# Gadersd/stable-diffusion-xl-burn

Hardware: NVIDIA H100
Metric: unet_sampler_steps_per_sec_1024x1024_bs1 (higher is better)
Workload: dtype f16

## Files before the change

### stable-diffusion-xl-burn_b200/csrc/attention.cu

```cuda
#include <stdlib.h>

#include "common.cuh"
#include "kernels.h"

namespace sdxl {

static constexpr int kTileBytes = 128 * 128;
static constexpr int kKvStages = 3;
static constexpr int kConsumerWarps = 8;
static constexpr int kAttnThreads = kConsumerWarps * 32 + 32;
static constexpr int kAttnSmem = 1024  + kTileBytes + 2 * kKvStages * kTileBytes + 256;

__device__ __forceinline__ float ex2_approx(float x) {
  float y;
  asm("ex2.approx.ftz.f32 %0, %1;" : "=f"(y) : "f"(x));
  return y;
}
__device__ __forceinline__ uint32_t pack_half2(float a, float b) {
  __half2 t = __floats2half2_rn(a, b);
  return *reinterpret_cast<uint32_t*>(&t);
}

__global__ void __launch_bounds__(kAttnThreads, 1) attention_kernel(const __grid_constant__ AttnParams p) {
  extern __shared__ uint8_t smem_raw[];
  uint8_t* smem = reinterpret_cast<uint8_t*>((reinterpret_cast<uintptr_t>(smem_raw) + 1023) & ~uintptr_t(1023));
  uint8_t* sQ = smem;
  uint8_t* sK = sQ + kTileBytes;
  uint8_t* sV = sK + kKvStages * kTileBytes;
  uint64_t* bars = reinterpret_cast<uint64_t*>(sV + kKvStages * kTileBytes);
  uint64_t* q_full = bars;
  uint64_t* kv_full = q_full + 1;
  uint64_t* kv_empty = kv_full + kKvStages;

  const int warp = threadIdx.x >> 5, lane = threadIdx.x & 31;
  const int nblk = (p.S + 127) / 128;
  const int nqt = (p.T + 127) / 128;
  const int qt = blockIdx.x % nqt, head = (blockIdx.x / nqt) % p.n_head, b = blockIdx.x / (nqt * p.n_head);

  if (threadIdx.x == 0) {
    tma_prefetch_desc(&p.tmQ);
    tma_prefetch_desc(&p.tmK);
    tma_prefetch_desc(&p.tmV);
    mbar_init(q_full, 1);
    for (int i = 0; i < kKvStages; ++i) { mbar_init(&kv_full[i], 1); mbar_init(&kv_empty[i], kConsumerWarps); }
    fence_barrier_init();
  }
  __syncthreads();
  griddep_wait();
  griddep_launch_dependents();

  if (warp == kConsumerWarps) {
    if (lane != 0) return;
    mbar_expect_tx(q_full, kTileBytes);
    tma_load_3d(sQ, &p.tmQ, q_full, p.q_col0 + head * 64, qt * 128, b);
    for (int j = 0; j < nblk; ++j) {
      const int st = j % kKvStages;
      mbar_wait_nocall(&kv_empty[st], ((j / kKvStages) & 1) ^ 1);
      mbar_expect_tx(&kv_full[st], 2 * kTileBytes);
      tma_load_3d(sK + st * kTileBytes, &p.tmK, &kv_full[st], p.k_col0 + head * 64, j * 128, b);
      tma_load_3d(sV + st * kTileBytes, &p.tmV, &kv_full[st], p.v_col0 + head * 64, j * 128, b);
    }
    return;
  }

  const int wg = warp >> 2;
  const float sl2e = p.scale_log2e;
  const uint32_t q_addr = smem_u32(sQ) + (uint32_t)wg * (64 * 128);
  float o[32];
#pragma unroll
  for (int i = 0; i < 32; ++i) o[i] = 0.f;
  float m[2] = {-INFINITY, -INFINITY}, l[2] = {0.f, 0.f};
  mbar_wait_nocall(q_full, 0);
  for (int j = 0; j < nblk; ++j) {
    const int st = j % kKvStages;
    mbar_wait_nocall(&kv_full[st], (j / kKvStages) & 1);
    float s[64];
    wg_fence();
    const uint32_t k_addr = smem_u32(sK + st * kTileBytes);
#pragma unroll
    for (int k = 0; k < 4; ++k) wgmma_ss_n128(s, wg_desc_sw128(q_addr + 32 * k), wg_desc_sw128(k_addr + 32 * k), k);
    wg_commit();
    wg_wait<0>();
    if (j * 128 + 128 > p.S) {
#pragma unroll
      for (int jj = 0; jj < 16; ++jj)
#pragma unroll
        for (int e = 0; e < 2; ++e)
          if (j * 128 + 8 * jj + 2 * (lane & 3) + e >= p.S) { s[4 * jj + e] = -INFINITY; s[4 * jj + 2 + e] = -INFINITY; }
    }
    uint32_t pa[32];
#pragma unroll
    for (int h = 0; h < 2; ++h) {
      float mx = -INFINITY;
#pragma unroll
      for (int jj = 0; jj < 16; ++jj) mx = fmaxf(mx, fmaxf(s[4 * jj + 2 * h], s[4 * jj + 2 * h + 1]));
      mx = fmaxf(mx, __shfl_xor_sync(0xffffffffu, mx, 1));
      mx = fmaxf(mx, __shfl_xor_sync(0xffffffffu, mx, 2));
      const float m_new = fmaxf(m[h], mx);
      const float alpha = ex2_approx((m[h] - m_new) * sl2e);
      const float mb = m_new * sl2e;
      float sum = 0.f;
#pragma unroll
      for (int jj = 0; jj < 16; ++jj) {
        const float p0 = ex2_approx(fmaf(s[4 * jj + 2 * h], sl2e, -mb));
        const float p1 = ex2_approx(fmaf(s[4 * jj + 2 * h + 1], sl2e, -mb));
        sum += p0 + p1;
        pa[4 * (jj >> 1) + 2 * (jj & 1) + h] = pack_half2(p0, p1);
      }
      l[h] = l[h] * alpha + sum;
      m[h] = m_new;
#pragma unroll
      for (int jj = 0; jj < 8; ++jj) { o[4 * jj + 2 * h] *= alpha; o[4 * jj + 2 * h + 1] *= alpha; }
    }
    wg_fence();
    const uint32_t v_addr = smem_u32(sV + st * kTileBytes);
#pragma unroll
    for (int kk = 0; kk < 8; ++kk)
      wgmma_rs_n64_tb(o, *reinterpret_cast<const uint32_t(*)[4]>(pa + 4 * kk), wg_desc_sw128(v_addr + 2048 * kk));
    wg_commit();
    wg_wait<0>();
    if (lane == 0) mbar_arrive(&kv_empty[st]);
  }
  const int r = wg * 64 + (warp & 3) * 16 + (lane >> 2);
#pragma unroll
  for (int h = 0; h < 2; ++h) {
    float lt = l[h];
    lt += __shfl_xor_sync(0xffffffffu, lt, 1);
    lt += __shfl_xor_sync(0xffffffffu, lt, 2);
    const float inv = 1.0f / lt;
    const int t = qt * 128 + r + 8 * h;
    if (t < p.T) {
      __half* out = p.out + ((size_t)b * p.T + t) * p.ldo + head * 64 + 2 * (lane & 3);
#pragma unroll
      for (int jj = 0; jj < 8; ++jj)
        *reinterpret_cast<__half2*>(out + 8 * jj) = __floats2half2_rn(o[4 * jj + 2 * h] * inv, o[4 * jj + 2 * h + 1] * inv);
    }
  }
}

static bool g_attn_attr[64];
int attention_launch(cudaStream_t st, const AttnParams& p) {
  if (p.T < 1 || p.S < 1 || (p.ldo & 1)) return 2002;
  int r = smem_optin(attention_kernel, kAttnSmem, g_attn_attr);
  if (r) return r;
  const long tiles = (long)p.B * p.n_head * ((p.T + 127) / 128);
  return launch_kernel(attention_kernel, dim3((unsigned)tiles), dim3(kAttnThreads), (size_t)kAttnSmem, st, true, p);
}

}
```

Before: 27.62.

## Make attention persistent with double-buffered Q and overlapped QK/PV wgmma

Turns the attention kernel into a persistent kernel sized to the SM count. It double-buffers Q tiles and keeps K/V resident across consecutive query tiles when the key length fits in one block (cross-attention). Inside the key loop, the next QK^T wgmma is issued alongside the previous block's PV wgmma so softmax overlaps tensor-core work. It also widens the producer to a full warpgroup with setmaxnreg rebalancing and adds a fourth KV stage, at the cost of more shared memory and more complex barrier phase tracking.

```diff
diff --git a/stable-diffusion-xl-burn_b200/csrc/attention.cu b/stable-diffusion-xl-burn_b200/csrc/attention.cu
--- a/stable-diffusion-xl-burn_b200/csrc/attention.cu
+++ b/stable-diffusion-xl-burn_b200/csrc/attention.cu
@@ -6,10 +6,9 @@
 namespace sdxl {
 
 static constexpr int kTileBytes = 128 * 128;
-static constexpr int kKvStages = 3;
-static constexpr int kConsumerWarps = 8;
-static constexpr int kAttnThreads = kConsumerWarps * 32 + 32;
-static constexpr int kAttnSmem = 1024  + kTileBytes + 2 * kKvStages * kTileBytes + 256;
+static constexpr int kKvStages = 4;
+static constexpr int kAttnThreads = 3 * 128;
+static constexpr int kAttnSmem = 1024  + 2 * kTileBytes + 2 * kKvStages * kTileBytes + 256;
 
 __device__ __forceinline__ float ex2_approx(float x) {
   float y;
@@ -21,27 +20,99 @@
   return *reinterpret_cast<uint32_t*>(&t);
 }
 
+__device__ __forceinline__ void softmax_block(float (&s)[64], float (&m)[2], float (&l)[2], float (&alpha)[2], int j, int S,
+                                              float sl2e, int lane) {
+  if (j * 128 + 128 > S) {
+#pragma unroll
+    for (int jj = 0; jj < 16; ++jj)
+#pragma unroll
+      for (int e = 0; e < 2; ++e)
+        if (j * 128 + 8 * jj + 2 * (lane & 3) + e >= S) { s[4 * jj + e] = -INFINITY; s[4 * jj + 2 + e] = -INFINITY; }
+  }
+#pragma unroll
+  for (int h = 0; h < 2; ++h) {
+    float mx = -INFINITY;
+#pragma unroll
+    for (int jj = 0; jj < 16; ++jj) mx = fmaxf(mx, fmaxf(s[4 * jj + 2 * h], s[4 * jj + 2 * h + 1]));
+    mx = fmaxf(mx, __shfl_xor_sync(0xffffffffu, mx, 1));
+    mx = fmaxf(mx, __shfl_xor_sync(0xffffffffu, mx, 2));
+    const float m_new = fmaxf(m[h], mx);
+    alpha[h] = ex2_approx((m[h] - m_new) * sl2e);
+    const float mb = m_new * sl2e;
+    float sum = 0.f;
+#pragma unroll
+    for (int jj = 0; jj < 16; ++jj) {
+      const float p0 = ex2_approx(fmaf(s[4 * jj + 2 * h], sl2e, -mb));
+      const float p1 = ex2_approx(fmaf(s[4 * jj + 2 * h + 1], sl2e, -mb));
+      sum += p0 + p1;
+      s[4 * jj + 2 * h] = p0;
+      s[4 * jj + 2 * h + 1] = p1;
+    }
+    l[h] = l[h] * alpha[h] + sum;
+    m[h] = m_new;
+  }
+}
+__device__ __forceinline__ void rescale_pack(float (&o)[32], const float (&s)[64], uint32_t (&pa)[32], const float (&alpha)[2]) {
+#pragma unroll
+  for (int h = 0; h < 2; ++h) {
+#pragma unroll
+    for (int jj = 0; jj < 8; ++jj) { o[4 * jj + 2 * h] *= alpha[h]; o[4 * jj + 2 * h + 1] *= alpha[h]; }
+#pragma unroll
+    for (int jj = 0; jj < 16; ++jj) pa[4 * (jj >> 1) + 2 * (jj & 1) + h] = pack_half2(s[4 * jj + 2 * h], s[4 * jj + 2 * h + 1]);
+  }
+}
+__device__ __forceinline__ void issue_s(float (&s)[64], uint32_t q_addr, uint32_t k_addr) {
+#pragma unroll
+  for (int k = 0; k < 4; ++k) wgmma_ss_n128(s, wg_desc_sw128(q_addr + 32 * k), wg_desc_sw128(k_addr + 32 * k), k);
+  wg_commit();
+}
+__device__ __forceinline__ void issue_pv(float (&o)[32], const uint32_t (&pa)[32], uint32_t v_addr) {
+#pragma unroll
+  for (int kk = 0; kk < 8; ++kk)
+    wgmma_rs_n64_tb(o, *reinterpret_cast<const uint32_t(*)[4]>(pa + 4 * kk), wg_desc_sw128(v_addr + 2048 * kk));
+  wg_commit();
+}
+
+struct TileWalk {
+  int nblk, nqt, t0, end, step;
+  bool resident;
+  __device__ TileWalk(const AttnParams& p) {
+    nblk = (p.S + 127) / 128;
+    nqt = (p.T + 127) / 128;
+    resident = nblk == 1;
+    const int tiles = p.B * p.n_head * nqt;
+    if (resident) {
+      t0 = (int)((long long)blockIdx.x * tiles / gridDim.x);
+      end = (int)((long long)(blockIdx.x + 1) * tiles / gridDim.x);
+      step = 1;
+    } else {
+      t0 = blockIdx.x;
+      end = tiles;
+      step = gridDim.x;
+    }
+  }
+};
+
 __global__ void __launch_bounds__(kAttnThreads, 1) attention_kernel(const __grid_constant__ AttnParams p) {
   extern __shared__ uint8_t smem_raw[];
   uint8_t* smem = reinterpret_cast<uint8_t*>((reinterpret_cast<uintptr_t>(smem_raw) + 1023) & ~uintptr_t(1023));
   uint8_t* sQ = smem;
-  uint8_t* sK = sQ + kTileBytes;
+  uint8_t* sK = sQ + 2 * kTileBytes;
   uint8_t* sV = sK + kKvStages * kTileBytes;
   uint64_t* bars = reinterpret_cast<uint64_t*>(sV + kKvStages * kTileBytes);
   uint64_t* q_full = bars;
-  uint64_t* kv_full = q_full + 1;
+  uint64_t* q_empty = q_full + 2;
+  uint64_t* kv_full = q_empty + 2;
   uint64_t* kv_empty = kv_full + kKvStages;
+  constexpr int kConsumerWarps = 8;
 
   const int warp = threadIdx.x >> 5, lane = threadIdx.x & 31;
-  const int nblk = (p.S + 127) / 128;
-  const int nqt = (p.T + 127) / 128;
-  const int qt = blockIdx.x % nqt, head = (blockIdx.x / nqt) % p.n_head, b = blockIdx.x / (nqt * p.n_head);
 
   if (threadIdx.x == 0) {
     tma_prefetch_desc(&p.tmQ);
     tma_prefetch_desc(&p.tmK);
     tma_prefetch_desc(&p.tmV);
-    mbar_init(q_full, 1);
+    for (int i = 0; i < 2; ++i) { mbar_init(&q_full[i], 1); mbar_init(&q_empty[i], kConsumerWarps); }
     for (int i = 0; i < kKvStages; ++i) { mbar_init(&kv_full[i], 1); mbar_init(&kv_empty[i], kConsumerWarps); }
     fence_barrier_init();
   }
@@ -49,102 +120,116 @@
   griddep_wait();
   griddep_launch_dependents();
 
-  if (warp == kConsumerWarps) {
-    if (lane != 0) return;
-    mbar_expect_tx(q_full, kTileBytes);
-    tma_load_3d(sQ, &p.tmQ, q_full, p.q_col0 + head * 64, qt * 128, b);
-    for (int j = 0; j < nblk; ++j) {
-      const int st = j % kKvStages;
-      mbar_wait_nocall(&kv_empty[st], ((j / kKvStages) & 1) ^ 1);
-      mbar_expect_tx(&kv_full[st], 2 * kTileBytes);
-      tma_load_3d(sK + st * kTileBytes, &p.tmK, &kv_full[st], p.k_col0 + head * 64, j * 128, b);
-      tma_load_3d(sV + st * kTileBytes, &p.tmV, &kv_full[st], p.v_col0 + head * 64, j * 128, b);
+  if (warp < 4) {
+    setmaxnreg_dec<24>();
+    if (warp != 0 || lane != 0) return;
+    const TileWalk walk(p);
+    const int nblk = walk.nblk, nqt = walk.nqt;
+    const bool resident = walk.resident;
+    uint32_t fill = 0;
+    int prev_bh = -1;
+    for (int t = walk.t0, i = 0; t < walk.end; t += walk.step, ++i) {
+      const int qt = t % nqt, bh = t / nqt, head = bh % p.n_head, b = bh / p.n_head;
+      mbar_wait_nocall(&q_empty[i & 1], ((i >> 1) & 1) ^ 1);
+      mbar_expect_tx(&q_full[i & 1], kTileBytes);
+      tma_load_3d(sQ + (i & 1) * kTileBytes, &p.tmQ, &q_full[i & 1], p.q_col0 + head * 64, qt * 128, b);
+      if (resident && bh == prev_bh) continue;
+      prev_bh = bh;
+      for (int j = 0; j < nblk; ++j, ++fill) {
+        const int st = fill % kKvStages;
+        mbar_wait_nocall(&kv_empty[st], ((fill / kKvStages) & 1) ^ 1);
+        mbar_expect_tx(&kv_full[st], 2 * kTileBytes);
+        tma_load_3d(sK + st * kTileBytes, &p.tmK, &kv_full[st], p.k_col0 + head * 64, j * 128, b);
+        tma_load_3d(sV + st * kTileBytes, &p.tmV, &kv_full[st], p.v_col0 + head * 64, j * 128, b);
+      }
     }
     return;
   }
 
-  const int wg = warp >> 2;
+  setmaxnreg_inc<240>();
+  const TileWalk walk(p);
+  const int nblk = walk.nblk, nqt = walk.nqt;
+  const bool resident = walk.resident;
+  const int wg = (warp >> 2) - 1;
   const float sl2e = p.scale_log2e;
-  const uint32_t q_addr = smem_u32(sQ) + (uint32_t)wg * (64 * 128);
-  float o[32];
-#pragma unroll
-  for (int i = 0; i < 32; ++i) o[i] = 0.f;
-  float m[2] = {-INFINITY, -INFINITY}, l[2] = {0.f, 0.f};
-  mbar_wait_nocall(q_full, 0);
-  for (int j = 0; j < nblk; ++j) {
-    const int st = j % kKvStages;
-    mbar_wait_nocall(&kv_full[st], (j / kKvStages) & 1);
+  const uint32_t sK0 = smem_u32(sK), sV0 = smem_u32(sV);
+  uint32_t next_fill = 0, kv0 = 0;
+  int prev_bh = -1;
+  for (int t = walk.t0, i = 0; t < walk.end; t += walk.step, ++i) {
+    const int qt = t % nqt, bh = t / nqt, head = bh % p.n_head, b = bh / p.n_head;
+    if (!(resident && bh == prev_bh)) { kv0 = next_fill; next_fill += nblk; }
+    prev_bh = bh;
+    const bool keep_kv = resident && t + walk.step < walk.end && (t + walk.step) / nqt == bh;
+    const uint32_t q_addr = smem_u32(sQ + (i & 1) * kTileBytes) + (uint32_t)wg * (64 * 128);
+    float o[32];
+#pragma unroll
+    for (int k = 0; k < 32; ++k) o[k] = 0.f;
+    float m[2] = {-INFINITY, -INFINITY}, l[2] = {0.f, 0.f}, alpha[2];
     float s[64];
+    uint32_t pa[32];
+    mbar_wait_nocall(&q_full[i & 1], (i >> 1) & 1);
+
+    uint32_t st = kv0 % kKvStages;
+    mbar_wait_nocall(&kv_full[st], (kv0 / kKvStages) & 1);
     wg_fence();
-    const uint32_t k_addr = smem_u32(sK + st * kTileBytes);
-#pragma unroll
-    for (int k = 0; k < 4; ++k) wgmma_ss_n128(s, wg_desc_sw128(q_addr + 32 * k), wg_desc_sw128(k_addr + 32 * k), k);
-    wg_commit();
+    issue_s(s, q_addr, sK0 + st * kTileBytes);
     wg_wait<0>();
-    if (j * 128 + 128 > p.S) {
-#pragma unroll
-      for (int jj = 0; jj < 16; ++jj)
-#pragma unroll
-        for (int e = 0; e < 2; ++e)
-          if (j * 128 + 8 * jj + 2 * (lane & 3) + e >= p.S) { s[4 * jj + e] = -INFINITY; s[4 * jj + 2 + e] = -INFINITY; }
-    }
-    uint32_t pa[32];
+    softmax_block(s, m, l, alpha, 0, p.S, sl2e, lane);
+    rescale_pack(o, s, pa, alpha);
+    if (nblk > 1) mbar_wait_nocall(&kv_full[(kv0 + 1) % kKvStages], ((kv0 + 1) / kKvStages) & 1);
+    for (int j = 1; j < nblk; ++j) {
+      const uint32_t f = kv0 + j, prev = st;
+      st = f % kKvStages;
+      wg_fence();
+      issue_s(s, q_addr, sK0 + st * kTileBytes);
+      issue_pv(o, pa, sV0 + prev * kTileBytes);
+      wg_wait<1>();
+      softmax_block(s, m, l, alpha, j, p.S, sl2e, lane);
+      if (j + 1 < nblk) mbar_wait_nocall(&kv_full[(f + 1) % kKvStages], ((f + 1) / kKvStages) & 1);
+      wg_wait<0>();
+      if (lane == 0) mbar_arrive(&kv_empty[prev]);
+      rescale_pack(o, s, pa, alpha);
+    }
+    wg_fence();
+    issue_pv(o, pa, sV0 + st * kTileBytes);
+    wg_wait<0>();
+    if (lane == 0) {
+      if (!keep_kv) mbar_arrive(&kv_empty[st]);
+      mbar_arrive(&q_empty[i & 1]);
+    }
+    const int r = wg * 64 + (warp & 3) * 16 + (lane >> 2);
 #pragma unroll
     for (int h = 0; h < 2; ++h) {
-      float mx = -INFINITY;
-#pragma unroll
-      for (int jj = 0; jj < 16; ++jj) mx = fmaxf(mx, fmaxf(s[4 * jj + 2 * h], s[4 * jj + 2 * h + 1]));
-      mx = fmaxf(mx, __shfl_xor_sync(0xffffffffu, mx, 1));
-      mx = fmaxf(mx, __shfl_xor_sync(0xffffffffu, mx, 2));
-      const float m_new = fmaxf(m[h], mx);
-      const float alpha = ex2_approx((m[h] - m_new) * sl2e);
-      const float mb = m_new * sl2e;
-      float sum = 0.f;
-#pragma unroll
-      for (int jj = 0; jj < 16; ++jj) {
-        const float p0 = ex2_approx(fmaf(s[4 * jj + 2 * h], sl2e, -mb));
-        const float p1 = ex2_approx(fmaf(s[4 * jj + 2 * h + 1], sl2e, -mb));
-        sum += p0 + p1;
-        pa[4 * (jj >> 1) + 2 * (jj & 1) + h] = pack_half2(p0, p1);
+      float lt = l[h];
+      lt += __shfl_xor_sync(0xffffffffu, lt, 1);
+      lt += __shfl_xor_sync(0xffffffffu, lt, 2);
+      const float inv = 1.0f / lt;
+      const int tq = qt * 128 + r + 8 * h;
+      if (tq < p.T) {
+        __half* out = p.out + ((size_t)b * p.T + tq) * p.ldo + head * 64 + 2 * (lane & 3);
+#pragma unroll
+        for (int jj = 0; jj < 8; ++jj)
+          *reinterpret_cast<__half2*>(out + 8 * jj) = __floats2half2_rn(o[4 * jj + 2 * h] * inv, o[4 * jj + 2 * h + 1] * inv);
       }
-      l[h] = l[h] * alpha + sum;
-      m[h] = m_new;
-#pragma unroll
-      for (int jj = 0; jj < 8; ++jj) { o[4 * jj + 2 * h] *= alpha; o[4 * jj + 2 * h + 1] *= alpha; }
-    }
-    wg_fence();
-    const uint32_t v_addr = smem_u32(sV + st * kTileBytes);
-#pragma unroll
-    for (int kk = 0; kk < 8; ++kk)
-      wgmma_rs_n64_tb(o, *reinterpret_cast<const uint32_t(*)[4]>(pa + 4 * kk), wg_desc_sw128(v_addr + 2048 * kk));
-    wg_commit();
-    wg_wait<0>();
-    if (lane == 0) mbar_arrive(&kv_empty[st]);
-  }
-  const int r = wg * 64 + (warp & 3) * 16 + (lane >> 2);
-#pragma unroll
-  for (int h = 0; h < 2; ++h) {
-    float lt = l[h];
-    lt += __shfl_xor_sync(0xffffffffu, lt, 1);
-    lt += __shfl_xor_sync(0xffffffffu, lt, 2);
-    const float inv = 1.0f / lt;
-    const int t = qt * 128 + r + 8 * h;
-    if (t < p.T) {
-      __half* out = p.out + ((size_t)b * p.T + t) * p.ldo + head * 64 + 2 * (lane & 3);
-#pragma unroll
-      for (int jj = 0; jj < 8; ++jj)
-        *reinterpret_cast<__half2*>(out + 8 * jj) = __floats2half2_rn(o[4 * jj + 2 * h] * inv, o[4 * jj + 2 * h + 1] * inv);
     }
   }
 }
 
 static bool g_attn_attr[64];
+static int g_attn_sms[64];
 int attention_launch(cudaStream_t st, const AttnParams& p) {
   if (p.T < 1 || p.S < 1 || (p.ldo & 1)) return 2002;
   int r = smem_optin(attention_kernel, kAttnSmem, g_attn_attr);
   if (r) return r;
+  int dev = 0;
+  if (cudaGetDevice(&dev) != cudaSuccess || dev < 0 || dev >= 64) return 2003;
+  if (!g_attn_sms[dev] && (cudaDeviceGetAttribute(&g_attn_sms[dev], cudaDevAttrMultiProcessorCount, dev) != cudaSuccess ||
+                           g_attn_sms[dev] <= 0))
+    return 2003;
   const long tiles = (long)p.B * p.n_head * ((p.T + 127) / 128);
-  return launch_kernel(attention_kernel, dim3((unsigned)tiles), dim3(kAttnThreads), (size_t)kAttnSmem, st, true, p);
-}
-
-}
+  if (tiles >= (1L << 31)) return 2002;
+  const long grid = tiles < g_attn_sms[dev] ? tiles : g_attn_sms[dev];
+  return launch_kernel(attention_kernel, dim3((unsigned)grid), dim3(kAttnThreads), (size_t)kAttnSmem, st, true, p);
+}
+
+}
```

Result: no change. 27.66 (median of 6 runs) (+0.2%).
